# reesque/SfmFromScratch

Measured on AMD Instinct MI355X. Metric: images/sec detect+describe+match, 1080p, 1/2/4/8 MI355X, higher is better.
Workload: dtype f32; 1 GPU; BASELINE configs[1]: 32x 1080p per GPU, ScaleRotInvSIFT 4-level x2 octave pyramid, k=2500, fw 18, NNRatio 0.85 over consecutive pairs; frames_per_gpu=32, pairs_per_gpu=31, distinct_batches=2, parallelism=image-shard x1, batches_in_flight=2

## Files before the change

include/sfmfeat.h:

```cpp
#ifndef SFMFEAT_H_
#define SFMFEAT_H_

#include <stddef.h>
#include <stdint.h>

#ifdef __cplusplus
extern "C" {
#endif

#define SFM_OK 0
#define SFM_EINVAL 1
#define SFM_ESTATE 2
#define SFM_EDEVICE 3
#define SFM_ERANGE 4
#define SFM_EINDEX 5

#define SFM_MODE_SCALEROT 0
#define SFM_MODE_NAIVE 1

#define SFM_DESC_DIM 128
#define SFM_MAX_GAUSS 15
#define SFM_MAX_KSIZE 31
#define SFM_MAX_FW 64
#define SFM_MAX_LEVELS 12
// ... 215 lines not shown
#define SFM_GEOM_COMPOSE 4
#define SFM_GEOM_ROTATE 5
#define SFM_GEOM_WAVE_SUM 6
#define SFM_GEOM_BLOCK_SUM 7
#define SFM_GEOM_OPS 8
int32_t sfm_debug_geom(int32_t device, int32_t op, const double* in, int64_t n, double* out);

int32_t sfm_debug_nms(int32_t device, const float* R, int32_t B, int32_t H, int32_t W, int32_t ksize,
                      const uint32_t* tnms, int32_t tile, uint64_t* keys_out, int64_t* counts_out);

#define SFM_SELECT_STATE_WORDS 11
#define SFM_SELECT_CONSTS 5
int32_t sfm_debug_select(int32_t device, int32_t nlevels, int32_t B, const float* const* R, const int32_t* H,
                         const int32_t* W, const int32_t* half_window, int32_t k, int32_t ksize, int64_t vmin,
                         int32_t force_exact, int32_t* x, int32_t* y, float* conf, int32_t* count,
                         uint32_t* state, int64_t* ncand, int32_t* consts);

float sfm_debug_time_harris(int32_t device, int32_t abl, int32_t B, int32_t H, int32_t W,
                            int32_t iters);
float sfm_debug_harris_stamps(int32_t device, int32_t abl, int32_t B, int32_t H, int32_t W,
                              int32_t iters, uint64_t* out, int64_t cap);

int64_t sfm_debug_match_stamps(uint64_t* out, int64_t cap);

int32_t sfm_debug_match_operands(sfm_ctx* ctx, int32_t slot, int64_t rows, uint16_t* hi, uint16_t* lo,
                                 float* norm2, float* rnorm, float* pmax);
int32_t sfm_debug_match_windows(sfm_ctx* ctx, int32_t pair, int64_t rows, int32_t* cand_n, float* cand_thr,
                                uint32_t* cand);
int32_t sfm_debug_match_skips(sfm_ctx* ctx, int32_t pair, int64_t rows, uint8_t* skip);

int32_t sfm_copy_wg(void* dst, const void* src, int64_t bytes, int32_t workgroups, void* stream);

int32_t sfm_debug_select_stats(sfm_ctx* ctx, int32_t* fallback_planes, int32_t* total_planes);
int32_t sfm_debug_pose_candidates(sfm_ctx* ctx, int32_t* cand_idx, int64_t entries);
int32_t sfm_debug_ransac_fits(sfm_ctx* ctx, double* F, int32_t* counts, int64_t entries);
int32_t sfm_debug_pnp_fits(sfm_ctx* ctx, double* hyp, int32_t* counts, double* start_Rt, int64_t entries);
int32_t sfm_debug_copy_level(sfm_ctx* ctx, int32_t l, int32_t what, float* out, void* stream);
int64_t sfm_debug_bmax_stride(int32_t h, int32_t w);
void sfm_debug_set_nms_blocks(int32_t mode);
int32_t sfm_debug_nms_blocks_rule(int32_t h, int32_t w, int32_t kcap, int32_t ksize);
int32_t sfm_debug_nms_blocks(int32_t device, const float* R, int32_t B, int32_t H, int32_t W, const uint32_t* tnms,
                             const uint32_t* fallback, int32_t blocks, int32_t inflate, uint64_t* keys_out,
                             int64_t* counts_out);


#ifdef __cplusplus
}
#endif

#endif
```

sfmfromscratch_amd/_native.py:

```python
from __future__ import annotations

import ctypes
import os
import sys
import threading

import numpy as np

from . import _abi
from ._abi import SfmParams

_HERE = os.path.dirname(os.path.abspath(__file__))
LIB_PATH = os.environ.get("SFMFEAT_LIB", os.path.join(_HERE, "lib", "libsfmfeat.so"))

_lib = None
_lib_lock = threading.Lock()

_fp = ctypes.POINTER(ctypes.c_float)
_i64p = ctypes.POINTER(ctypes.c_int64)
_i32p = ctypes.POINTER(ctypes.c_int32)
_u8p = ctypes.POINTER(ctypes.c_uint8)
_dp = ctypes.POINTER(ctypes.c_double)
_vp = ctypes.c_void_p

# ... 56 lines not shown
                                               _vp, _vp, _vp, _vp, _vp, _vp, ctypes.c_double, _vp, _vp, _vp]),
    "sfm_resect_tracks_dev": (ctypes.c_int32, [_vp, _vp, _vp, ctypes.c_int32, ctypes.c_int64, _vp, _vp,
                                               ctypes.c_int32, _vp, _vp, ctypes.c_int32, ctypes.c_double,
                                               ctypes.c_int32, ctypes.c_int64, ctypes.c_int32, _vp, _vp, _vp, _vp,
                                               _vp, _vp, _vp]),
    "sfm_ingest_rgb_dev": (ctypes.c_int32, [_vp, _vp, ctypes.c_int32, ctypes.c_int32, ctypes.c_int32,
                                            ctypes.c_int32, ctypes.c_int32, _vp, _vp]),
    "sfm_extract_batch_dev": (ctypes.c_int32, [_vp, _vp, ctypes.c_int32, ctypes.c_int32, ctypes.c_int32, _vp, _vp,
                                               _vp, ctypes.c_int64, _vp]),
    "sfm_extract_batch_u8_dev": (ctypes.c_int32, [_vp, _vp, ctypes.c_int32, ctypes.c_int32, ctypes.c_int32, _vp,
                                                  _vp, _vp, ctypes.c_int64, _vp]),
    "sfm_match_pairs_dev": (ctypes.c_int32, [_vp, _vp, _vp, ctypes.c_int32, ctypes.c_int64, _vp, ctypes.c_int32,
                                             ctypes.c_float, _vp, _vp, _vp, _vp]),
    "sfm_match_prep_dev": (ctypes.c_int32, [_vp, _vp, _vp, ctypes.c_int32, ctypes.c_int64, ctypes.c_int32,
                                            ctypes.c_int32, _vp]),
    "sfm_match_pairs_prepped_dev": (ctypes.c_int32, [_vp, _vp, _vp, ctypes.c_int32, ctypes.c_int64, _vp,
                                                     ctypes.c_int32, ctypes.c_float, _vp, _vp, _vp, _vp]),
    "sfm_ctx_stream": (ctypes.c_int32, [_vp, ctypes.POINTER(_vp)]),
    "sfm_ctx_set_serial": (ctypes.c_int32, [_vp, ctypes.c_int32]),
    "sfm_ctx_set_fused_prep": (ctypes.c_int32, [_vp, ctypes.c_int32]),
    "sfm_ctx_set_priority": (ctypes.c_int32, [_vp, ctypes.c_int32]),
    "sfm_gate_create": (ctypes.c_int32, [ctypes.c_int32, ctypes.POINTER(_vp)]),
    "sfm_gate_destroy": (ctypes.c_int32, [_vp]),
    "sfm_ctx_set_gate": (ctypes.c_int32, [_vp, _vp]),
    "sfm_profile_enable": (ctypes.c_int32, [_vp, ctypes.c_int32]),
    "sfm_profile_stages": (ctypes.c_int32, [_vp, ctypes.c_int32]),
    "sfm_profile_read": (ctypes.c_int32, [_vp, ctypes.POINTER(ctypes.c_double), _i64p, ctypes.c_int32]),
    "sfm_profile_spans": (ctypes.c_int32, [_vp, ctypes.c_int64]),
    "sfm_profile_spans_read": (ctypes.c_int32, [_vp, _i64p, _i32p, ctypes.c_int64, _i64p, _i64p, ctypes.c_int32]),
    "sfm_debug_time_harris": (ctypes.c_float, [ctypes.c_int32] * 6),
    "sfm_debug_harris_stamps": (ctypes.c_float, [ctypes.c_int32] * 6 + [ctypes.c_void_p, ctypes.c_int64]),
    "sfm_debug_match_stamps": (ctypes.c_int64, [ctypes.c_void_p, ctypes.c_int64]),
    "sfm_debug_select_stats": (ctypes.c_int32, [_vp, _i32p, _i32p]),
    **_abi.MATCH_DEBUG_SIGNATURES,
    **_abi.GEOM_DEBUG_SIGNATURES,
    **_abi.SELECT_DEBUG_SIGNATURES,
    **_abi.PNP_DEBUG_SIGNATURES,
    "sfm_copy_wg": (ctypes.c_int32, [_vp, _vp, ctypes.c_int64, ctypes.c_int32, _vp]),
    "sfm_dist_unique_id": (ctypes.c_int32, [_u8p]),
    "sfm_dist_create": (ctypes.c_int32, [ctypes.c_int32, ctypes.c_int32, ctypes.c_int32, _u8p, ctypes.POINTER(_vp)]),
    "sfm_dist_destroy": (ctypes.c_int32, [_vp]),
    "sfm_dist_last_error": (ctypes.c_char_p, [_vp]),
    "sfm_dist_rank": (ctypes.c_int32, [_vp, _i32p, _i32p]),
    "sfm_dist_allgather_slots_dev": (ctypes.c_int32, [_vp, ctypes.c_int32, ctypes.c_int32, _vp, _vp, _vp, _vp, _vp,
                                                      _vp, ctypes.c_int64, _vp]),
    "sfm_dist_halo_dev": (ctypes.c_int32, [_vp, ctypes.c_int32, _vp, _vp, _vp, _vp, _vp, _vp, _vp]),

    "sfm_debug_copy_level": (ctypes.c_int32, [_vp, ctypes.c_int32, ctypes.c_int32, _vp, _vp]),
    "sfm_debug_atan2": (ctypes.c_int32, [ctypes.c_int32, _fp, _fp, _fp, ctypes.c_int64]),
    "sfm_debug_harris": (ctypes.c_int32, [ctypes.c_int32, _fp, ctypes.c_int32, ctypes.c_double, ctypes.c_int32,
                                          _fp, ctypes.c_int32, ctypes.c_int32, _fp, _fp, _i64p]),
    "sfm_debug_nms": (ctypes.c_int32, [ctypes.c_int32, _fp, ctypes.c_int32, ctypes.c_int32, ctypes.c_int32,
                                       ctypes.c_int32, _vp, ctypes.c_int32, _vp, _i64p]),
    "sfm_debug_bmax_stride": (ctypes.c_int64, [ctypes.c_int32, ctypes.c_int32]),
    "sfm_debug_set_nms_blocks": (None, [ctypes.c_int32]),
    "sfm_debug_nms_blocks_rule": (ctypes.c_int32, [ctypes.c_int32] * 4),
    "sfm_debug_nms_blocks": (ctypes.c_int32, [ctypes.c_int32, _fp, ctypes.c_int32, ctypes.c_int32, ctypes.c_int32,
                                              _vp, _vp, ctypes.c_int32, ctypes.c_int32, _vp, _i64p]),
}


class NativeLibraryMissing(ImportError):
    pass


def _preload_torch_hip_runtime():
# ... 94 lines not shown
            raise RuntimeError("sfm_ctx_create failed: no usable MI355X (HIP) device")
        self.handle = h
        self.capacity = int(self.lib.sfm_keypoint_capacity(ctypes.byref(params)))
        self.levels = 1 if params.mode == _abi.SFM_MODE_NAIVE else int(params.pyramid_level)

    def close(self):
        if getattr(self, "handle", None) is not None and self.handle.value:
            self.lib.sfm_ctx_destroy(self.handle)
            self.handle = _vp()

    def __del__(self):
        try:
            self.close()
        except Exception:
            pass

    def stream(self) -> int:
        h = _vp()
        check(self.lib.sfm_ctx_stream(self.handle, ctypes.byref(h)), self.handle)
        return int(h.value or 0)

    def set_priority(self, priority: int):
        check(self.lib.sfm_ctx_set_priority(self.handle, int(priority)), self.handle)

    def set_fused_prep(self, on: bool):
        check(self.lib.sfm_ctx_set_fused_prep(self.handle, 1 if on else 0), self.handle)

    def set_serial(self, serial: bool):
        check(self.lib.sfm_ctx_set_serial(self.handle, 1 if serial else 0), self.handle)

    def select_stats(self):
        fb, tot = ctypes.c_int32(0), ctypes.c_int32(0)
        check(self.lib.sfm_debug_select_stats(self.handle, ctypes.byref(fb), ctypes.byref(tot)), self.handle)
        return int(fb.value), int(tot.value)

    def copy_level(self, level: int, what: int, out_ptr: int, stream: int):
        check(self.lib.sfm_debug_copy_level(self.handle, int(level), int(what), ctypes.c_void_p(out_ptr),
                                            ctypes.c_void_p(stream)), self.handle)

    def extract(self, img: np.ndarray):
        if img.dtype != np.float32:
            img = img.astype(np.float32)
        if img.strides[1] != 4:
            img = np.ascontiguousarray(img)
        H, W = img.shape
        cap = max(self.capacity, 1)
        X = np.empty(cap, np.int64)
        Y = np.empty(cap, np.int64)
        D = np.empty((cap, 128), np.float32)
        C = np.empty(cap, np.float32)
        lc = np.zeros(self.levels, np.int32)
        n = ctypes.c_int64(0)
        rc = self.lib.sfm_extract(self.handle, img.ctypes.data_as(_fp), H, W, img.strides[0] // 4,
                                  X.ctypes.data_as(_i64p), Y.ctypes.data_as(_i64p), D.ctypes.data_as(_fp),
                                  C.ctypes.data_as(_fp), cap, ctypes.byref(n), lc.ctypes.data_as(_i32p))
        check(rc, self.handle)
        k = n.value
        return X[:k], Y[:k], D[:k], C[:k], lc

    def match(self, d1: np.ndarray, d2: np.ndarray, ratio32: np.float32):
        d1 = np.ascontiguousarray(d1, dtype=np.float32)
        d2 = np.ascontiguousarray(d2, dtype=np.float32)
        n1, n2 = d1.shape[0], d2.shape[0]
        cap = max(n1, 1)
        m = np.empty((cap, 2), np.int64)
        c = np.empty(cap, np.float32)
# ... 306 lines not shown
    nc = ctypes.c_int64(0)
    check(load_library().sfm_debug_harris(device, g.ctypes.data_as(_fp), gs, params.alpha, params.ksize,
                                          img.ctypes.data_as(_fp), H, W, R.ctypes.data_as(_fp),
                                          med.ctypes.data_as(_fp), ctypes.byref(nc)))
    return R, med[0], nc.value


def debug_nms(R: np.ndarray, tnms, ksize: int = 3, tile: bool = False, device: int = 0):
    R = np.ascontiguousarray(R, dtype=np.float32)
    B, H, W = R.shape
    t = np.ascontiguousarray(tnms, dtype=np.uint32)
    keys = np.zeros(B * H * W, np.uint64)
    cnt = np.zeros(B, np.int64)
    check(load_library().sfm_debug_nms(device, R.ctypes.data_as(_fp), B, H, W, ksize, t.ctypes.data,
                                       int(tile), keys.ctypes.data, cnt.ctypes.data_as(_i64p)))
    return [np.sort(keys[b * H * W: b * H * W + cnt[b]]) for b in range(B)]


def debug_nms_blocks(R: np.ndarray, tnms, fallback=None, blocks: bool = True, inflate: bool = False, device: int = 0):
    R = np.ascontiguousarray(R, dtype=np.float32)
    B, H, W = R.shape
    t = np.ascontiguousarray(tnms, dtype=np.uint32)
    fb = np.zeros(B, np.uint32) if fallback is None else np.ascontiguousarray(fallback, dtype=np.uint32)
    assert t.shape == (B,) and fb.shape == (B,)
    keys = np.zeros(B * H * W, np.uint64)
    cnt = np.zeros(B, np.int64)
    check(load_library().sfm_debug_nms_blocks(device, R.ctypes.data_as(_fp), B, H, W, t.ctypes.data, fb.ctypes.data,
                                              int(blocks), int(inflate), keys.ctypes.data, cnt.ctypes.data_as(_i64p)))
    return [np.sort(keys[b * H * W: b * H * W + cnt[b]]) for b in range(B)]


def set_nms_blocks(mode: int):
    load_library().sfm_debug_set_nms_blocks(int(mode))


def nms_blocks_rule(h: int, w: int, kcap: int, ksize: int = 3) -> bool:
    return bool(load_library().sfm_debug_nms_blocks_rule(int(h), int(w), int(kcap), int(ksize)))


def bmax_stride(h: int, w: int) -> int:
    return int(load_library().sfm_debug_bmax_stride(int(h), int(w)))


def debug_geom(op: int, rows: np.ndarray, device: int = 0) -> np.ndarray:
    op = int(op)
    if not 0 <= op < len(_abi.GEOM_ROW_IN):
        raise ValueError(f"debug_geom: unknown op {op}")
    if not isinstance(rows, np.ndarray) or rows.dtype != np.float64 or not rows.flags.c_contiguous:
        raise ValueError("debug_geom: rows must be a C-contiguous float64 array")
    if rows.ndim != 2 or rows.shape[1] != _abi.GEOM_ROW_IN[op]:
        raise ValueError(f"debug_geom: op {op} takes rows of {_abi.GEOM_ROW_IN[op]} values, got shape {rows.shape}")
    n = rows.shape[0]
    if n > _abi.SFM_GEOM_MAX_ROWS:
        raise ValueError(f"debug_geom: at most {_abi.SFM_GEOM_MAX_ROWS} rows")
    out = np.empty((n, _abi.GEOM_ROW_OUT[op]), np.float64)
    if n:
        check(load_library().sfm_debug_geom(device, op, rows.ctypes.data, n, out.ctypes.data))
    return out


def select_constants(k: int) -> dict:
    consts = np.zeros(_abi.SFM_SELECT_CONSTS, np.int32)
    check(load_library().sfm_debug_select(0, 0, 0, None, None, None, None, int(k), 1, 0, 0, None, None, None, None,
                                          None, None, consts.ctypes.data))
    return dict(zip(_abi.SELECT_CONST_FIELDS, consts.tolist()))

# ... 147 lines not shown
```

sfmfromscratch_amd/csrc/api_extract.hip:

```cpp
#include "ctx.h"

using namespace sfm;

static_assert(kLayoutMedBins == kMedBins1 && kLayoutCounterStride == kCounterStride &&
                  kLayoutMedianStateBytes == sizeof(MedianState) && kLayoutSelectMaxLevels == kSelectMaxLevels,
              "extract_layout.h mirrors kernels.h");
static_assert(layout_bmax_stride(1080, 1920) == bmax_plane_stride(1080, 1920) &&
                  layout_bmax_stride(270, 480) == bmax_plane_stride(270, 480) &&
                  layout_bmax_stride(70, 132) == bmax_plane_stride(70, 132),
              "extract_layout.h mirrors kernels.h");

static int g_nms_blocks_override = -2;
void extract_set_nms_blocks(int mode) { g_nms_blocks_override = mode < -1 ? -2 : mode; }

LayoutSwitches extract_layout_switches() {
  LayoutSwitches s = extract_switches().layout;
  if (g_nms_blocks_override != -2) s.nms_blocks = g_nms_blocks_override;
  return s;
}

const ExtractSwitches& extract_switches() {
  static const ExtractSwitches sw = [] {
    ExtractSwitches s;
    s.layout.pyr_fused = env_int(getenv("SFMFEAT_PYR_FUSED"), 1) != 0;
// ... 112 lines not shown
    const float alpha = (float)c->p.alpha;
    if (!(l0 > 0 && (skip & 16))) launch_harris_levels(g, B, as<float>(c->ex.gauss), c->p.gaussian_size, alpha, st);
  }

  void select_level(int l, hipStream_t s) {
    StageScope sc(c, SFM_PROF_TOPK, s);
    if (skip & 1) return;
    launch_select(R(l), cand(l), candcnt + y.counter[l], at<uint32_t>(kBufMedlist, y.sel[l]),
                  at<uint64_t>(kBufScratch, y.sel[l]), kp(l), std::max(c->kcap, 1), c->kcap, B, y.lv[l].h, y.lv[l].w,
                  c->p.ksize, y.lv[l].fw / 2, med(l), s);
  }

  void select_merged() {
    StageScope sc(c, SFM_PROF_TOPK, st);
    SelectLevels g{};
    g.n = y.L - y.L_aux;
    for (int l = y.L_aux; l < y.L; ++l)
      g.l[l - y.L_aux] = SelectLevels::Level{R(l), cand(l), candcnt + y.counter[l], at<uint32_t>(kBufMedlist, y.sel[l]),
                                             at<uint64_t>(kBufScratch, y.sel[l]), kp(l), med(l), y.lv[l].h, y.lv[l].w,
                                             y.lv[l].fw / 2};
    if (!(skip & 1)) launch_select_levels(g, std::max(c->kcap, 1), c->kcap, B, c->p.ksize, st);
  }

  void describe_level(int l, hipStream_t s) {
    StageScope sc(c, SFM_PROF_DESCRIBE, s);
    const int L = y.L;
    if ((skip & 2) && l != L - 1) {
      fused_ok = false;
      return;
    }
    bool ow = false;
    const bool r = launch_describe(lvl[l], B, y.lv[l].h, y.lv[l].w, y.lv[l].fw, c->p.mode == SFM_MODE_NAIVE ? 0 : 1,
                                   kp(l), c->kcap, as<int32_t>(c->ex.buf[kBufLc]), l, L, y.lv[l].scale, xy, desc, conf,
                                   cap, l == L - 1 ? count : nullptr, mo, &ow, s);
    if (l == L - 1) counted = r;
    fused_ok = fused_ok && ow;
  }

  int release_gate() {
    if (c->gate && !gate_released) {
      HIPCHK(c, hipEventRecord(c->gate->ev, st));
      c->gate->armed = true;
      gate_released = true;
    }
    return SFM_OK;
  }

  int run(const float* imgs);
};

int Extraction::run(const float* imgs) {
  const int L = y.L, L_aux = y.L_aux;
  CtxStreams& cs = c->s;
  int rc;
  lvl[0] = imgs;
  for (int l = 1; l < L; ++l) lvl[l] = at<float>(kBufLvl, y.lvl[l]);
  zeroed = sw.fill_launches;
  {
    StageScope sc(c, SFM_PROF_PYRAMID, st);
    if (!y.pyr_fused) pyramid_from(1);
  }
  if ((rc = operands_fused_begin(c, desc, count, cap, B, &mo))) return rc;
  if (mo.hi) HIPCHK(c, hipMemsetAsync(mo.pmax, 0, (size_t)B * match_pmax_bytes(mo.capP), st));
  fused_ok = mo.hi != nullptr;
  if (!zeroed || sw.fill_launches) {
    HIPCHK(c, hipMemsetAsync(c->ex.buf[kBufHist].p, 0, y.bytes[kBufHist], st));
    HIPCHK(c, hipMemsetAsync(c->ex.buf[kBufCounts].p, 0, y.bytes[kBufCounts], st));
// ... 158 lines not shown
```

sfmfromscratch_amd/csrc/api_profile.hip:

```cpp
#include "ctx.h"

using namespace sfm;

namespace {

int spans_reset(sfm_ctx* c) {
  ProfilerWs& pr = c->prof;
  pr.span_n = 0;
  pr.span_dropped = 0;
  pr.span_level.clear();
  if (pr.span_cap == 0) return SFM_OK;
  std::vector<unsigned long long> init((size_t)2 * pr.span_cap, 0ull);
  for (int64_t i = 0; i < pr.span_cap; ++i) init[2 * i] = ~0ull;
  HIPCHK(c, hipDeviceSynchronize());
  HIPCHK(c, hipMemcpy(pr.spans.p, init.data(), init.size() * 8, hipMemcpyHostToDevice));
  return SFM_OK;
}

}

extern "C" {

int32_t sfm_profile_enable(sfm_ctx* c, int32_t on) {
  if (!c) return SFM_EINVAL;
// ... 72 lines not shown
int32_t sfm_debug_copy_level(sfm_ctx* c, int32_t l, int32_t what, float* out, void* stream) {
  if (!c || !out || l < 0 || l >= c->L || !c->ex.last_B) return SFM_EINVAL;
  ExtractWs& x = c->ex;
  ExtractLayout y;
  if (extract_layout(&c->p, c->kcap, x.last_B, x.last_H, x.last_W, c->serial, extract_layout_switches(), &y) != SFM_OK)
    return SFM_EINVAL;
  if (what == 2) {
    if (!((x.last_mapped >> l) & 1u) || y.bmax[l] < 0) return set_err(c, SFM_EINVAL, "the level wrote no block-maximum map");
    HIPCHK(c, hipMemcpyAsync(out, as<float>(x.buf[kBufBmax]) + y.bmax[l],
                             (size_t)x.last_B * bmax_plane_stride(y.lv[l].h, y.lv[l].w) * 4, hipMemcpyDeviceToDevice,
                             (hipStream_t)stream));
    return SFM_OK;
  }
  const size_t bytes = (size_t)x.last_B * y.lv[l].h * y.lv[l].w * 4;
  const float* src = what == 0 ? as<float>(x.buf[kBufR]) + y.plane[l]
                               : (l == 0 ? as<float>(x.buf[kBufImg0]) : as<float>(x.buf[kBufLvl]) + y.lvl[l]);
  HIPCHK(c, hipMemcpyAsync(out, src, bytes, hipMemcpyDeviceToDevice, (hipStream_t)stream));
  return SFM_OK;
}

int32_t sfm_debug_select_stats(sfm_ctx* c, int32_t* fallback_planes, int32_t* total_planes) {
  if (!c || !fallback_planes || !total_planes) return SFM_EINVAL;
  *fallback_planes = 0;
  *total_planes = c->L * c->ex.last_B;
  if (*total_planes == 0) return SFM_OK;
  HIPCHK(c, hipSetDevice(c->device));
  HIPCHK(c, hipDeviceSynchronize());
  std::vector<MedianState> ms((size_t)*total_planes);
  HIPCHK(c, hipMemcpy(ms.data(), c->ex.buf[kBufMed].p, ms.size() * sizeof(MedianState), hipMemcpyDeviceToHost));
  for (const MedianState& m : ms) *fallback_planes += m.fallback ? 1 : 0;
  return SFM_OK;
}

}
```

sfmfromscratch_amd/csrc/debug.hip:

```cpp
#include <string.h>

#include <vector>

#include "../../include/sfmfeat.h"
#include "kernels.h"

using namespace sfm;

namespace sfm {

__global__ void k_debug_atan2(const float* __restrict__ y, const float* __restrict__ x,
                              float* __restrict__ out, int64_t n) {
  int64_t i = (int64_t)blockIdx.x * blockDim.x + threadIdx.x;
  if (i < n) out[i] = svml_atan2f(y[i], x[i]);
}

__global__ void __launch_bounds__(256) k_copy_wg(const uint4* __restrict__ src, uint4* __restrict__ dst, int64_t n16,
                                                 const uint8_t* __restrict__ src_b, uint8_t* __restrict__ dst_b,
                                                 int64_t tail) {
  const int64_t stride = (int64_t)gridDim.x * blockDim.x;
  for (int64_t i = (int64_t)blockIdx.x * blockDim.x + threadIdx.x; i < n16; i += stride) dst[i] = src[i];
  if (blockIdx.x == 0 && threadIdx.x < tail) dst_b[threadIdx.x] = src_b[threadIdx.x];
}

// ... 122 lines not shown
    x = x * 1664525u + 1013904223u;
    h[i] = (float)(x >> 24) / 255.0f;
  }
  float g0[49];
  for (int i = 0; i < 49; ++i) g0[i] = 1.0f / 49.0f;
  std::vector<float> g(harris_taps_floats(7));
  harris_taps_build(g0, 7, g.data());
  (void)hipMemcpy(d_img, h.data(), n * 4, hipMemcpyHostToDevice);
  (void)hipMemcpy(d_g, g.data(), 4 * g.size(), hipMemcpyHostToDevice);
  (void)hipMemset(d_hist, 0, (size_t)B * 4 * kMedBins1);
  float ms = time_harris_ablation(abl, d_img, d_R, d_hist, B, H, W, d_g, 0.05f, iters, d_st, d_st ? cap : 0);
  if (d_st) {
    (void)hipMemcpy(out, d_st, (size_t)cap * 8, hipMemcpyDeviceToHost);
    (void)hipFree(d_st);
  }
  void* bufs[] = {d_img, d_R, d_g, d_hist};
  for (void* b : bufs) (void)hipFree(b);
  return ms;
}

int32_t sfm_copy_wg(void* dst, const void* src, int64_t bytes, int32_t workgroups, void* stream) {
  if (bytes < 0 || workgroups < 1 || (bytes > 0 && (!dst || !src))) return SFM_EINVAL;
  if ((((uintptr_t)dst) | ((uintptr_t)src)) & 15) return SFM_EINVAL;
  if (bytes == 0) return SFM_OK;
  const int64_t n16 = bytes / 16, tail = bytes - 16 * n16;
  hipLaunchKernelGGL(k_copy_wg, dim3((unsigned)workgroups), dim3(256), 0, (hipStream_t)stream,
                     (const uint4*)src, (uint4*)dst, n16, (const uint8_t*)src + 16 * n16, (uint8_t*)dst + 16 * n16,
                     tail);
  return hipGetLastError() == hipSuccess ? SFM_OK : SFM_EDEVICE;
}

int64_t sfm_debug_match_stamps(uint64_t* out, int64_t cap) { return sfm::match_stamps_copy(out, cap); }

}
```

sfmfromscratch_amd/csrc/describe.hip:

```cpp
#include "kernels.h"

#include <stdlib.h>

namespace sfm {

SFM_DEV double pi_edge(int i, int num) {
  const double start = -3.141592653589793, stop = 3.141592653589793;
  if (i == num - 1) return stop;
  double step = (stop - start) / (double)(num - 1);
  return (double)i * step + start;
}

struct DescLayout {
  int ws, n, n4, pw, P;
  size_t off_keys, off_patch, off_ori, off_mag, off_sw, off_cw, off_cellw, off_wgh, total;
};

__host__ __device__ inline DescLayout desc_layout(int fw, int rotate) {
  DescLayout L;
  int h = fw / 2;
  L.ws = 2 * h;
  L.n = L.ws * L.ws;
  L.pw = L.ws + 2;
  int P = 1;
// ... 231 lines not shown
  float v0 = w0, v1 = w1;
  if (nrm > 0.0f) {
    v0 = v0 / nrm;
    v1 = v1 / nrm;
  }
  out_desc[slot * 128 + lane] = sqrtf(v0);
  out_desc[slot * 128 + lane + 64] = sqrtf(v1);
  if (lane == 0) {
    if (out_conf) out_conf[slot] = kp.conf[ko];
    out_xy[slot * 2 + 0] = (int32_t)((double)x * scale);
    out_xy[slot * 2 + 1] = (int32_t)((double)y * scale);
  }
}

__global__ void k_finalize_counts(const int32_t* __restrict__ lc_all, int B, int L,
                                  int32_t* __restrict__ out_count) {
  int b = blockIdx.x * blockDim.x + threadIdx.x;
  if (b >= B) return;
  int32_t s = 0;
  for (int l = 0; l < L; ++l) s += lc_all[(int64_t)l * B + b];
  out_count[b] = s;
}

size_t describe_lds_bytes(int fw, int rotate) { return desc_layout(fw, rotate).total; }

void init_describe_attributes(size_t max_lds) {
  (void)hipFuncSetAttribute((const void*)k_describe, hipFuncAttributeMaxDynamicSharedMemorySize,
                            (int)max_lds);
}

bool launch_describe(const float* lvl, int B, int H, int W, int fw, int rotate, KpList kp,
                     int kcap, const int32_t* level_counts_all, int level, int L, double scale,
                     int32_t* out_xy, float* out_desc, float* out_conf, int64_t out_cap,
                     int32_t* out_count, const MatchOperands& mo, bool* operands_written, hipStream_t st) {
  if (operands_written) *operands_written = false;
  if (kcap <= 0) return false;
  static const bool one_per_wave = [] {
    const char* v = getenv("SFMFEAT_DESCRIBE");
    return v && v[0] == 'w';
  }();
  if (!one_per_wave && launch_describe_quad(lvl, B, H, W, fw, rotate, kp, kcap, level_counts_all, level,
                                            scale, out_xy, out_desc, out_conf, out_cap, out_count, L, mo, st)) {
    if (operands_written) *operands_written = mo.hi != nullptr;
    return out_count != nullptr;
  }
  size_t lds = describe_lds_bytes(fw, rotate);
  hipLaunchKernelGGL(k_describe, dim3(kcap, B), dim3(64), lds, st, lvl, H, W, fw, rotate, kp, kcap,
                     level_counts_all, level, B, scale, out_xy, out_desc, out_conf, out_cap);
  return false;
}

void launch_finalize_counts(const int32_t* level_counts_all, int B, int L, int32_t* out_count,
                            hipStream_t st) {
  hipLaunchKernelGGL(k_finalize_counts, dim3((B + 255) / 256), dim3(256), 0, st, level_counts_all, B, L,
                     out_count);
}

}
```

sfmfromscratch_amd/csrc/describe_q.hip:

```cpp
#include "kernels.h"

#include <stdlib.h>
#include <string.h>

#include <mutex>

namespace sfm {
namespace dq {

constexpr int cmax(int a, int b) { return a > b ? a : b; }
constexpr int pow2ceil(int v) { return v <= 1 ? 1 : 2 * pow2ceil((v + 1) / 2); }

template <int WS, int ROT>
struct Geo {
  static constexpr int N = WS * WS, PW = WS + 2, NP = PW * PW;
  static constexpr int P = cmax(pow2ceil(N), 16), E = P / 16;
  static constexpr int RN = (N + 15) / 16;
  static constexpr int A = (cmax(cmax(NP, N + 4), 16 * 17) + 3) & ~3;
  static constexpr int NQ = (N + 3) & ~3;
  static constexpr int OFF_M = A;
  static constexpr int OFF_K = OFF_M + NQ;
  static constexpr int OFF_R = OFF_K + NQ;
  static constexpr int OFF_I = OFF_R + (ROT ? (NQ / 2 + 3) & ~3 : 0);
  static constexpr int OFF_T = OFF_I + (ROT ? 40 : 0);
  static constexpr int G = OFF_T + 12;
};

SFM_DEV double pi_edge(int i, int num) {
  const double start = -3.141592653589793, stop = 3.141592653589793;
  if (i == num - 1) return stop;
  const double step = (stop - start) / (double)(num - 1);
  return (double)i * step + start;
}
// ... 113 lines not shown
  gy = __builtin_fmaf(-2.0f, a01, gy);
  gy = __builtin_fmaf(-1.0f, a02, gy);
  gy = __builtin_fmaf(1.0f, a20, gy);
  gy = __builtin_fmaf(2.0f, a21, gy);
  gy = __builtin_fmaf(1.0f, a22, gy);
  const float sx = gx * gx;
  const float sy = gy * gy;
  const float s = sx + sy;
  mag = sqrtf(s);
  ori = svml_atan2f(gy, gx);
}

SFM_DEV void cas_up(uint32_t& a, uint32_t& b) {
  const uint32_t lo = min(a, b), hi = max(a, b);
  a = lo;
  b = hi;
}

template <typename T>
SFM_DEV void batcher16(T (&q)[16]) {
#pragma unroll
  for (int p = 1; p < 16; p <<= 1)
#pragma unroll
    for (int kk = p; kk >= 1; kk >>= 1)
#pragma unroll
      for (int j = kk % p; j + kk < 16; j += 2 * kk)
#pragma unroll
        for (int i = 0; i < kk; ++i) {
          const int a = i + j, c = i + j + kk;
          if (c < 16 && a / (2 * p) == c / (2 * p)) cas_up(q[a], q[c]);
        }
}

template <int WS, int ROT, int ABL = 0>
__global__ void __launch_bounds__(64) k_describe_q(const float* __restrict__ lvl, int H, int W, KpList kp,
                                                   int kcap, const int32_t* __restrict__ lc_all, int level,
                                                   int B, double scale, int32_t* __restrict__ out_xy,
                                                   float* __restrict__ out_desc, float* __restrict__ out_conf,
                                                   int64_t out_cap, int32_t* __restrict__ out_count, int L,
                                                   MatchOperands mo) {
  using C = Geo<WS, ROT>;
  constexpr int N = C::N, PW = C::PW, NP = C::NP, E = C::E, RN = C::RN, h = WS / 2;
  __shared__ __attribute__((aligned(16))) float s_all[4 * C::G];
  const int b = blockIdx.y;
  if (out_count != nullptr && blockIdx.x == 0 && threadIdx.x == 0) {
    int32_t s = 0;
    for (int l = 0; l < L; ++l) s += lc_all[(int64_t)l * B + b];
    out_count[b] = s;
  }
  const int nkb = (kcap + 3) / 4;
  if ((int)blockIdx.x >= nkb) {
    int32_t s = 0;
    for (int l = 0; l < L; ++l) s += lc_all[(int64_t)l * B + b];
    const int nt = ((int)gridDim.x - nkb) * 64;
    for (int64_t r = s + ((int)blockIdx.x - nkb) * 64 + threadIdx.x; r < mo.capP; r += nt) {
      const int64_t mr = (int64_t)b * mo.capP + r;
      uint4* hz = reinterpret_cast<uint4*>(mo.hi + mr * 128);
      uint4* lz = reinterpret_cast<uint4*>(mo.lo + mr * 128);
#pragma unroll
      for (int q = 0; q < 16; ++q) {
        hz[q] = make_uint4(0u, 0u, 0u, 0u);
        lz[q] = make_uint4(0u, 0u, 0u, 0u);
      }
      mo.norm2[mr] = INFINITY;
      mo.rnorm[mr] = 0.0f;
    }
    return;
  }
  const int count = kp.count[b];
  const int kbase = blockIdx.x * 4;
  if (kbase >= count) return;
  const int lane = threadIdx.x, g = lane >> 4, gl = lane & 15;
  const int kpi = kbase + g;
  const bool valid = kpi < count;
  const int64_t ko = (int64_t)b * kcap + (valid ? kpi : kbase);
  const int x = kp.x[ko], y = kp.y[ko];
  float* sA = s_all + g * C::G;
  float* sM = sA + C::OFF_M;
  uint32_t* sK = reinterpret_cast<uint32_t*>(sA + C::OFF_K);
  uint16_t* sR = reinterpret_cast<uint16_t*>(sA + C::OFF_R);
  int32_t* sI = reinterpret_cast<int32_t*>(sA + C::OFF_I);
  uint32_t* sT = reinterpret_cast<uint32_t*>(sA + C::OFF_T);

  const float* img = lvl + (int64_t)b * H * W;
#pragma unroll
  for (int it = 0; it < (NP + 15) / 16; ++it) {
    const int e0 = it * 16 + gl;
    const int e = e0 < NP ? e0 : NP - 1;
    const int pr = e / PW, pc = e - pr * PW;
    const int gy = y - h + pr, gx = x - h + pc;
    const bool in = gy >= 0 && gy < H && gx >= 0 && gx < W;
    const int cy = min(max(gy, 0), H - 1), cx = min(max(gx, 0), W - 1);
    const float v = (ABL & 64) ? (float)(cy + cx) : img[(int64_t)cy * W + cx];
    if (e0 < NP) sA[e] = in ? v : 0.0f;
  }
  __syncthreads();

  double k[E];
  bool tiny = false;
#pragma unroll
  for (int r = 0; r < E; ++r) k[r] = __longlong_as_double((long long)kPad);
#pragma unroll
  for (int r = 0; r < RN; ++r) {
    const int e0 = r * 16 + gl;
    const bool ok = (N % 16 == 0) || e0 < N;
    const int e = ok ? e0 : N - 1;
    const int i = e / WS, j = e - i * WS;
    float mag, ori;
    if constexpr ((ABL & 8) != 0) {
      mag = sA[(i + 1) * PW + (j + 1)];
      ori = sA[(i + 1) * PW + j] - 100.0f;
    } else {
      grad_at(sA + (i + 1) * PW + (j + 1), PW, mag, ori);
    }
    if (ok) {
      sM[e] = mag;
      if (!ROT) sK[e] = __float_as_uint(ori);
    }
    if (ROT) {
      k[r] = ok ? dkey(((uint64_t)fkey(ori) << 9) | (uint32_t)e) : __longlong_as_double((long long)kPad);
      tiny |= ok && ori != 0.0f && fabsf(ori) < 0x1p-25f;
    }
  }
  __syncthreads();

  double dom = 0.0;
  int dom_bin = 36;
  if constexpr (ROT) {
    if constexpr ((ABL & 1) == 0) merge_level<E, 2>(k, gl);
    float w[E];
    uint32_t ke[E], kf[E];
#pragma unroll
    for (int r = 0; r < E; ++r) {
      const int p = gl * E + r;
      const uint64_t pl = dpayload(k[r]);
      ke[r] = p < N ? (uint32_t)(pl & 511u) : 0u;
      kf[r] = (uint32_t)(pl >> 9);
      w[r] = p < N ? sM[ke[r]] : 0.0f;
    }
    __syncthreads();
    float cw[E];
#pragma unroll
    for (int r = 0; r < E; ++r) cw[r] = 0.0f;
    float carry = 0.0f;
    constexpr int NL = (N + E - 1) / E;
    if constexpr ((ABL & 2) != 0) {
#pragma unroll
      for (int r = 0; r < E; ++r) cw[r] = w[r];
    }
    for (int s = 0; s < ((ABL & 2) ? 0 : NL); ++s) {
      if (gl == s) {
        float acc = carry;
#pragma unroll
        for (int r = 0; r < E; ++r) {
          acc = acc + w[r];
          cw[r] = acc;
        }
      }
      const float nxt = __uint_as_float(dpp<0x111>(__float_as_uint(cw[E - 1])));
      if (gl == s + 1) carry = nxt;
    }
// ... 44 lines not shown
    for (int t = 0; t < 3; ++t) {
      const int j = gl + 16 * t;
      if (j < 36) {
        const float v = sA[3 + sI[j + 1]] - sA[3 + sI[j]];
        if (v > hb) { hb = v; bi = j; }
      }
    }
    {
      float ov; int oi;
      ov = rxorf<8>(hb); oi = (int)rxor<8>((uint32_t)bi);
      if (ov > hb || (ov == hb && oi < bi)) { hb = ov; bi = oi; }
      ov = rxorf<4>(hb); oi = (int)rxor<4>((uint32_t)bi);
      if (ov > hb || (ov == hb && oi < bi)) { hb = ov; bi = oi; }
      ov = rxorf<2>(hb); oi = (int)rxor<2>((uint32_t)bi);
      if (ov > hb || (ov == hb && oi < bi)) { hb = ov; bi = oi; }
      ov = rxorf<1>(hb); oi = (int)rxor<1>((uint32_t)bi);
      if (ov > hb || (ov == hb && oi < bi)) { hb = ov; bi = oi; }
    }
    dom = (pi_edge(bi, 37) + pi_edge(bi + 1, 37)) / 2.0;
    dom_bin = bi;
  }

  if (gl < 9) sT[gl] = (ABL & 32) ? 0x80000000u + (uint32_t)(dom * 1e6) * gl : c_cell[dom_bin][gl];
  __syncthreads();
  float hv[8];
  if constexpr ((ABL & 4) != 0) {
#pragma unroll
    for (int bb = 0; bb < 8; ++bb) hv[bb] = sM[gl * 8 + bb] + __uint_as_float(sT[bb & 7]);
  } else {
  const int r4 = gl >> 2, c4 = gl & 3;
  float wv[16];
  uint32_t hk[16];
  const bool grp_tiny = ROT && ((__ballot(tiny) >> (16 * g)) & 0xFFFFull) != 0;
  if (ROT && !grp_tiny) {
    uint32_t q[16];
#pragma unroll
    for (int t = 0; t < 16; ++t) {
      const int i = 4 * r4 + (t >> 2), j = 4 * c4 + (t & 3);
      const bool ok = i < WS && j < WS;
      q[t] = ok ? (uint32_t)sR[ok ? i * WS + j : 0] : 0xFFFFFFFFu;
    }
    batcher16(q);
#pragma unroll
    for (int m = 0; m < 16; ++m) {
      const bool ok = q[m] != 0xFFFFFFFFu;
      const uint32_t p = ok ? q[m] : 0u;
      wv[m] = ok ? sM[p] : 0.0f;
      hk[m] = ok ? sK[p] : 0xFFFFFFFFu;
    }
  } else {
    uint64_t q[16];
#pragma unroll
    for (int t = 0; t < 16; ++t) {
      const int i = 4 * r4 + (t >> 2), j = 4 * c4 + (t & 3);
      const bool ok = i < WS && j < WS;
      const int e = ok ? i * WS + j : 0;
      const uint32_t key = ROT ? sK[sR[e]] : fkey(__uint_as_float(sK[e]));
      q[t] = ok ? (((uint64_t)key << 32) | (uint32_t)t) : ~0ull;
    }
    if (!ROT) {
      double dq16[16];
#pragma unroll
      for (int t = 0; t < 16; ++t) dq16[t] = q[t] == ~0ull ? __longlong_as_double((long long)kPad)
                                                           : dkey(((q[t] >> 32) << 4) | (uint32_t)t);
      batcher16(dq16);
#pragma unroll
      for (int t = 0; t < 16; ++t) {
// ... 130 lines not shown
namespace {
uint32_t fkey_h(float v) {
  uint32_t b;
  memcpy(&b, &v, 4);
  if (b == 0x80000000u) b = 0u;
  return (b & 0x80000000u) ? ~b : (b | 0x80000000u);
}
float fkey_inv_h(uint32_t k) {
  const uint32_t b = (k & 0x80000000u) ? (k & 0x7fffffffu) : ~k;
  float f;
  memcpy(&f, &b, 4);
  return f;
}
double pi_edge_h(int i, int num) {
  const double start = -3.141592653589793, stop = 3.141592653589793;
  if (i == num - 1) return stop;
  const double step = (stop - start) / (double)(num - 1);
  return (double)i * step + start;
}
uint32_t edge_key_h(double e, double sh, bool strict) {
  auto pass = [&](uint32_t kk) {
    const double d = (double)fkey_inv_h(kk) - sh;
    return strict ? d > e : d >= e;
  };
  uint32_t lo = fkey_h(-INFINITY), hi = fkey_h(INFINITY);
  while (hi - lo > 1u) {
    const uint32_t mid = lo + (hi - lo) / 2u;
    if (pass(mid)) hi = mid; else lo = mid;
  }
  return hi;
}
}

void init_describe_quad_tables() {
  static std::mutex mu;
  static bool done[256] = {};
  int dev = 0;
  if (hipGetDevice(&dev) != hipSuccess || dev < 0 || dev >= 256) return;
  std::lock_guard<std::mutex> lk(mu);
  if (done[dev]) return;
  uint32_t ori[37], cell[37][9];
  for (int j = 0; j < 37; ++j) ori[j] = edge_key_h(pi_edge_h(j, 37), 0.0, j == 36);
  for (int bi = 0; bi < 37; ++bi) {
    const double dom = bi < 36 ? (pi_edge_h(bi, 37) + pi_edge_h(bi + 1, 37)) / 2.0 : 0.0;
    for (int t = 0; t < 9; ++t) cell[bi][t] = edge_key_h(pi_edge_h(t, 9), dom, t == 8);
  }
  done[dev] = hipMemcpyToSymbol(HIP_SYMBOL(dq::c_ori), ori, sizeof(ori)) == hipSuccess &&
              hipMemcpyToSymbol(HIP_SYMBOL(dq::c_cell), cell, sizeof(cell)) == hipSuccess;
}

#define SFM_DQ_BODY(WS)                                                                              \
    if (rotate)                                                                                      \
      hipLaunchKernelGGL((dq::k_describe_q<WS, 1>), grid, dim3(64), 0, st, lvl, H, W, kp, kcap, lc,  \
                         level, B, scale, out_xy, out_desc, out_conf, out_cap, out_count, L, mo);        \
    else                                                                                             \
      hipLaunchKernelGGL((dq::k_describe_q<WS, 0>), grid, dim3(64), 0, st, lvl, H, W, kp, kcap, lc,  \
                         level, B, scale, out_xy, out_desc, out_conf, out_cap, out_count, L, mo);        \
    return true;
#define SFM_DQ_CASE(WS) \
  case WS:              \
    SFM_DQ_BODY(WS)

bool launch_describe_quad(const float* lvl, int B, int H, int W, int fw, int rotate, KpList kp, int kcap,
                          const int32_t* lc, int level, double scale, int32_t* out_xy, float* out_desc,
                          float* out_conf, int64_t out_cap, int32_t* out_count, int L, const MatchOperands& mo,
                          hipStream_t st) {
  constexpr int kPadBlocks = 8;
  const dim3 grid((kcap + 3) / 4 + (mo.hi != nullptr && out_count != nullptr ? kPadBlocks : 0), B);
  switch (2 * (fw / 2)) {
    SFM_DQ_CASE(2)
    SFM_DQ_CASE(4)
    SFM_DQ_CASE(6)
    SFM_DQ_CASE(8)
    SFM_DQ_CASE(10)
    SFM_DQ_CASE(12)
    SFM_DQ_CASE(14)
    SFM_DQ_CASE(16)
    case 18:
#ifdef SFM_ABLATIONS
      if (rotate) {
        static const int abl = [] {
          const char* v = SFM_ABLATION_ENV("SFMFEAT_DQ_ABL");
          return v ? atoi(v) : 0;
        }();
        switch (abl) {
#define SFM_DQ_ABL(A)                                                                                     \
  case A:                                                                                                \
    hipLaunchKernelGGL((dq::k_describe_q<18, 1, A>), grid, dim3(64), 0, st, lvl, H, W, kp, kcap, lc, level, \
                       B, scale, out_xy, out_desc, out_conf, out_cap, out_count, L, mo);                     \
    return true;
          SFM_DQ_ABL(1)
          SFM_DQ_ABL(2)
          SFM_DQ_ABL(4)
          SFM_DQ_ABL(8)
          SFM_DQ_ABL(7)
          SFM_DQ_ABL(16)
          SFM_DQ_ABL(32)
          SFM_DQ_ABL(64)
          SFM_DQ_ABL(55)
          SFM_DQ_ABL(127)
          default:
            break;
        }
      }
#endif
      SFM_DQ_BODY(18)
    SFM_DQ_CASE(20)
    SFM_DQ_CASE(22)
    default:
      return false;
  }
}

}
```

sfmfromscratch_amd/csrc/kernels.h:

```cpp
#pragma once

#include <hip/hip_runtime.h>
#include <stdint.h>

#include <vector>

#include "common.h"

namespace sfm {

#define SFM_NMS_MAX_HALF 15

constexpr int kHistBits = 12;
constexpr int kHistBins = 1 << kHistBits;
constexpr int kMedBits1 = 11;
constexpr int kMedBins1 = 1 << kMedBits1;
constexpr int kTopkLdsCap = 8192;
constexpr int kMaxMatchRows = 16384;
constexpr int kMatchCandCap = 256;
constexpr int kCounterStride = 32;
constexpr int kMatchUnitPairBits = 20;

constexpr float kMatchScale = 256.0f;
constexpr float kMatchLoScale = 2048.0f;
// ... 327 lines not shown

void launch_nms(const float* R, const MedianState* state, uint64_t* cand,
                unsigned long long* cand_count, int B, int H, int W, int ksize, int mode, hipStream_t st,
                int force_tile = 0, const float* bmax = nullptr);
bool nms_blocks_shape(int W, int ksize, int mode);

void init_topk_attributes();
void init_describe_attributes(size_t max_lds);
void init_describe_quad_tables();
size_t describe_lds_bytes(int fw, int rotate);
void launch_select(const float* R, uint64_t* cand, const unsigned long long* cand_count, uint32_t* medlist,
                   uint64_t* scratch, KpList kp, int kcap, int k, int B, int H, int W, int ksize, int half_window,
                   MedianState* state, hipStream_t st);
constexpr int kSelectMaxLevels = 4;
struct SelectLevels {
  struct Level {
    const float* R;
    uint64_t* cand;
    const unsigned long long* cand_count;
    uint32_t* medlist;
    uint64_t* scratch;
    KpList kp;
    MedianState* state;
    int H, W, hw;
  } l[kSelectMaxLevels];
  int n;
};
void launch_select_levels(const SelectLevels& g, int kcap, int k, int B, int ksize, hipStream_t st);
void select_branch_sizes(int k, int32_t out[5]);

bool launch_describe_quad(const float* lvl, int B, int H, int W, int fw, int rotate, KpList kp, int kcap,
                          const int32_t* level_counts_all, int level, double scale, int32_t* out_xy,
                          float* out_desc, float* out_conf, int64_t out_cap, int32_t* out_count, int L,
                          const MatchOperands& mo, hipStream_t st);
bool launch_describe(const float* lvl, int B, int H, int W, int fw, int rotate, KpList kp,
                     int kcap, const int32_t* level_counts_all, int level, int L, double scale,
                     int32_t* out_xy, float* out_desc, float* out_conf, int64_t out_cap,
                     int32_t* out_count, const MatchOperands& mo, bool* operands_written, hipStream_t st);
void launch_finalize_counts(const int32_t* level_counts_all, int B, int L, int32_t* out_count,
                            hipStream_t st);

struct RowBest {
  int32_t col;
  float nndr;
};
SFM_DEV void top2_update(float d, int j, float& e1, int& j1, float& e2) {
  if (d < e1 || (d == e1 && j < j1)) {
    e2 = e1;
    e1 = d;
    j1 = j;
  } else if (d < e2) {
    e2 = d;
  }
}
SFM_DEV void top2_merge(float& e1, int& j1, float& e2, float o1, int oj, float o2) {
  if (o1 < e1 || (o1 == e1 && oj < j1)) {
    e2 = fminf(e1, o2);
    e1 = o1;
    j1 = oj;
  } else {
    e2 = fminf(e2, o1);
  }
}
SFM_DEV RowBest top2_finish(float e1, int j1, float e2, float ratio) {
  RowBest rb;
  rb.col = -1;
  rb.nndr = 0.0f;
  const float d1 = sqrtf(e1), d2 = sqrtf(e2);
  if (d2 > 0.0f) {
    const float nndr = d1 / d2;
    if (nndr <= ratio) { rb.col = j1; rb.nndr = nndr; }
// ... 23 lines not shown
```

Before: 45080 images/sec.

## Certify dominant orientation via LDS histogram, skip full sort when margin safe

For rotation-invariant describe at widths 4 and 20+, each keypoint group builds a 36-bin orientation histogram in shared memory with atomics and finds the top two bins. If the gap between them exceeds a rounding-error bound for every group in the wave, the dominant bin is taken directly and the full merge-sort over all patch samples is skipped. Otherwise it falls back to the original sorted path and bumps a fallback counter. This adds histogram atomics, LDS traffic and a new per-cell sort on the fast path, and only applies to certain window widths.

```diff
diff --git a/include/sfmfeat.h b/include/sfmfeat.h
--- a/include/sfmfeat.h
+++ b/include/sfmfeat.h
@@ -271,6 +271,10 @@
 int32_t sfm_copy_wg(void* dst, const void* src, int64_t bytes, int32_t workgroups, void* stream);
 
 int32_t sfm_debug_select_stats(sfm_ctx* ctx, int32_t* fallback_planes, int32_t* total_planes);
+#define SFM_DESCRIBE_CERT_C 8
+#define SFM_DESCRIBE_CERT_TMIN_EXP (-64)
+void sfm_debug_set_describe_cert(int32_t mode);
+int32_t sfm_debug_describe_stats(sfm_ctx* ctx, int64_t* fallback_groups, int64_t* groups);
 int32_t sfm_debug_pose_candidates(sfm_ctx* ctx, int32_t* cand_idx, int64_t entries);
 int32_t sfm_debug_ransac_fits(sfm_ctx* ctx, double* F, int32_t* counts, int64_t entries);
 int32_t sfm_debug_pnp_fits(sfm_ctx* ctx, double* hyp, int32_t* counts, double* start_Rt, int64_t entries);
diff --git a/sfmfromscratch_amd/_native.py b/sfmfromscratch_amd/_native.py
--- a/sfmfromscratch_amd/_native.py
+++ b/sfmfromscratch_amd/_native.py
@@ -112,6 +112,8 @@
     "sfm_debug_harris_stamps": (ctypes.c_float, [ctypes.c_int32] * 6 + [ctypes.c_void_p, ctypes.c_int64]),
     "sfm_debug_match_stamps": (ctypes.c_int64, [ctypes.c_void_p, ctypes.c_int64]),
     "sfm_debug_select_stats": (ctypes.c_int32, [_vp, _i32p, _i32p]),
+    "sfm_debug_set_describe_cert": (None, [ctypes.c_int32]),
+    "sfm_debug_describe_stats": (ctypes.c_int32, [_vp, _i64p, _i64p]),
     **_abi.MATCH_DEBUG_SIGNATURES,
     **_abi.GEOM_DEBUG_SIGNATURES,
     **_abi.SELECT_DEBUG_SIGNATURES,
@@ -272,6 +274,11 @@
     def select_stats(self):
         fb, tot = ctypes.c_int32(0), ctypes.c_int32(0)
         check(self.lib.sfm_debug_select_stats(self.handle, ctypes.byref(fb), ctypes.byref(tot)), self.handle)
+        return int(fb.value), int(tot.value)
+
+    def describe_stats(self):
+        fb, tot = ctypes.c_int64(0), ctypes.c_int64(0)
+        check(self.lib.sfm_debug_describe_stats(self.handle, ctypes.byref(fb), ctypes.byref(tot)), self.handle)
         return int(fb.value), int(tot.value)
 
     def copy_level(self, level: int, what: int, out_ptr: int, stream: int):
@@ -644,6 +651,10 @@
 
 def set_nms_blocks(mode: int):
     load_library().sfm_debug_set_nms_blocks(int(mode))
+
+
+def set_describe_cert(mode: int):
+    load_library().sfm_debug_set_describe_cert(int(mode))
 
 
 def nms_blocks_rule(h: int, w: int, kcap: int, ksize: int = 3) -> bool:
diff --git a/sfmfromscratch_amd/csrc/api_extract.hip b/sfmfromscratch_amd/csrc/api_extract.hip
--- a/sfmfromscratch_amd/csrc/api_extract.hip
+++ b/sfmfromscratch_amd/csrc/api_extract.hip
@@ -168,7 +168,7 @@
     bool ow = false;
     const bool r = launch_describe(lvl[l], B, y.lv[l].h, y.lv[l].w, y.lv[l].fw, c->p.mode == SFM_MODE_NAIVE ? 0 : 1,
                                    kp(l), c->kcap, as<int32_t>(c->ex.buf[kBufLc]), l, L, y.lv[l].scale, xy, desc, conf,
-                                   cap, l == L - 1 ? count : nullptr, mo, &ow, s);
+                                   cap, l == L - 1 ? count : nullptr, mo, &ow, donecnt + y.counter[l], s);
     if (l == L - 1) counted = r;
     fused_ok = fused_ok && ow;
   }
diff --git a/sfmfromscratch_amd/csrc/api_profile.hip b/sfmfromscratch_amd/csrc/api_profile.hip
--- a/sfmfromscratch_amd/csrc/api_profile.hip
+++ b/sfmfromscratch_amd/csrc/api_profile.hip
@@ -128,4 +128,31 @@
   return SFM_OK;
 }
 
+int32_t sfm_debug_describe_stats(sfm_ctx* c, int64_t* fallback_groups, int64_t* groups) {
+  if (!c || !fallback_groups || !groups) return SFM_EINVAL;
+  *fallback_groups = *groups = 0;
+  ExtractWs& x = c->ex;
+  if (!x.last_B || c->p.mode == SFM_MODE_NAIVE) return SFM_OK;
+  ExtractLayout y;
+  if (extract_layout(&c->p, c->kcap, x.last_B, x.last_H, x.last_W, c->serial, extract_layout_switches(), &y) != SFM_OK)
+    return SFM_EINVAL;
+  HIPCHK(c, hipSetDevice(c->device));
+  HIPCHK(c, hipDeviceSynchronize());
+  const int B = x.last_B, L = y.L;
+  std::vector<int32_t> lc((size_t)L * B);
+  std::vector<unsigned long long> cnt((size_t)y.counter_block);
+  HIPCHK(c, hipMemcpy(lc.data(), x.buf[kBufLc].p, lc.size() * 4, hipMemcpyDeviceToHost));
+  HIPCHK(c, hipMemcpy(cnt.data(), as<unsigned long long>(x.buf[kBufCounts]) + 3 * y.counter_block, cnt.size() * 8,
+                      hipMemcpyDeviceToHost));
+  for (int l = 0; l < L; ++l) {
+    const int ws = 2 * (y.lv[l].fw / 2);
+    if (ws < 2 || ws > 22) continue;
+    for (int b = 0; b < B; ++b) {
+      *groups += (lc[(size_t)l * B + b] + 3) / 4;
+      *fallback_groups += (int64_t)cnt[(size_t)(y.counter[l] + (int64_t)b * kCounterStride + 1)];
+    }
+  }
+  return SFM_OK;
 }
+
+}
diff --git a/sfmfromscratch_amd/csrc/debug.hip b/sfmfromscratch_amd/csrc/debug.hip
--- a/sfmfromscratch_amd/csrc/debug.hip
+++ b/sfmfromscratch_amd/csrc/debug.hip
@@ -178,4 +178,6 @@
 
 int64_t sfm_debug_match_stamps(uint64_t* out, int64_t cap) { return sfm::match_stamps_copy(out, cap); }
 
+void sfm_debug_set_describe_cert(int32_t mode) { describe_set_cert(mode); }
+
 }
diff --git a/sfmfromscratch_amd/csrc/describe.hip b/sfmfromscratch_amd/csrc/describe.hip
--- a/sfmfromscratch_amd/csrc/describe.hip
+++ b/sfmfromscratch_amd/csrc/describe.hip
@@ -287,7 +287,8 @@
 bool launch_describe(const float* lvl, int B, int H, int W, int fw, int rotate, KpList kp,
                      int kcap, const int32_t* level_counts_all, int level, int L, double scale,
                      int32_t* out_xy, float* out_desc, float* out_conf, int64_t out_cap,
-                     int32_t* out_count, const MatchOperands& mo, bool* operands_written, hipStream_t st) {
+                     int32_t* out_count, const MatchOperands& mo, bool* operands_written,
+                     unsigned long long* fb_count, hipStream_t st) {
   if (operands_written) *operands_written = false;
   if (kcap <= 0) return false;
   static const bool one_per_wave = [] {
@@ -295,7 +296,8 @@
     return v && v[0] == 'w';
   }();
   if (!one_per_wave && launch_describe_quad(lvl, B, H, W, fw, rotate, kp, kcap, level_counts_all, level,
-                                            scale, out_xy, out_desc, out_conf, out_cap, out_count, L, mo, st)) {
+                                            scale, out_xy, out_desc, out_conf, out_cap, out_count, L, mo, fb_count,
+                                            st)) {
     if (operands_written) *operands_written = mo.hi != nullptr;
     return out_count != nullptr;
   }
diff --git a/sfmfromscratch_amd/csrc/describe_q.hip b/sfmfromscratch_amd/csrc/describe_q.hip
--- a/sfmfromscratch_amd/csrc/describe_q.hip
+++ b/sfmfromscratch_amd/csrc/describe_q.hip
@@ -1,4 +1,5 @@
 #include "kernels.h"
+#include "../../include/sfmfeat.h"
 
 #include <stdlib.h>
 #include <string.h>
@@ -178,16 +179,23 @@
         }
 }
 
+constexpr float kCertBoundPerN = (float)SFM_DESCRIBE_CERT_C * 0x1p-24f;
+constexpr uint32_t kCertTminBits = (uint32_t)(127 + SFM_DESCRIBE_CERT_TMIN_EXP) << 23;
+constexpr bool cert_width(int ws) { return ws == 4 || ws >= 20; }
+
 template <int WS, int ROT, int ABL = 0>
 __global__ void __launch_bounds__(64) k_describe_q(const float* __restrict__ lvl, int H, int W, KpList kp,
                                                    int kcap, const int32_t* __restrict__ lc_all, int level,
                                                    int B, double scale, int32_t* __restrict__ out_xy,
                                                    float* __restrict__ out_desc, float* __restrict__ out_conf,
                                                    int64_t out_cap, int32_t* __restrict__ out_count, int L,
-                                                   MatchOperands mo) {
+                                                   MatchOperands mo, int cert,
+                                                   unsigned long long* __restrict__ fb_count) {
   using C = Geo<WS, ROT>;
   constexpr int N = C::N, PW = C::PW, NP = C::NP, E = C::E, RN = C::RN, h = WS / 2;
+  constexpr bool CERT = ROT && (ABL == 128 || (ABL == 0 && cert_width(WS)));
   __shared__ __attribute__((aligned(16))) float s_all[4 * C::G];
+  __shared__ uint32_t s_ori[CERT ? 40 : 1];
   const int b = blockIdx.y;
   if (out_count != nullptr && blockIdx.x == 0 && threadIdx.x == 0) {
     int32_t s = 0;
@@ -226,6 +234,7 @@
   uint32_t* sK = reinterpret_cast<uint32_t*>(sA + C::OFF_K);
   uint16_t* sR = reinterpret_cast<uint16_t*>(sA + C::OFF_R);
   int32_t* sI = reinterpret_cast<int32_t*>(sA + C::OFF_I);
+  float* sH = sA + C::OFF_I;
   uint32_t* sT = reinterpret_cast<uint32_t*>(sA + C::OFF_T);
 
   const float* img = lvl + (int64_t)b * H * W;
@@ -240,12 +249,16 @@
     const float v = (ABL & 64) ? (float)(cy + cx) : img[(int64_t)cy * W + cx];
     if (e0 < NP) sA[e] = in ? v : 0.0f;
   }
+  if constexpr (CERT) {
+    if (lane < 37) s_ori[lane] = c_ori[lane];
+    sH[gl] = 0.0f;
+    sH[gl + 16] = 0.0f;
+    if (gl < 4) sH[gl + 32] = 0.0f;
+  }
   __syncthreads();
 
-  double k[E];
   bool tiny = false;
-#pragma unroll
-  for (int r = 0; r < E; ++r) k[r] = __longlong_as_double((long long)kPad);
+  float tsum = 0.0f;
 #pragma unroll
   for (int r = 0; r < RN; ++r) {
     const int e0 = r * 16 + gl;
@@ -261,18 +274,63 @@
     }
     if (ok) {
       sM[e] = mag;
-      if (!ROT) sK[e] = __float_as_uint(ori);
-    }
-    if (ROT) {
-      k[r] = ok ? dkey(((uint64_t)fkey(ori) << 9) | (uint32_t)e) : __longlong_as_double((long long)kPad);
-      tiny |= ok && ori != 0.0f && fabsf(ori) < 0x1p-25f;
+      sK[e] = ROT ? fkey(ori) : __float_as_uint(ori);
+    }
+    if (ROT) tiny |= ok && ori != 0.0f && fabsf(ori) < 0x1p-25f;
+    if constexpr (CERT) {
+      const uint32_t fk = fkey(ori);
+      const float t = (ori + __uint_as_float(0x40490fdbu)) * 5.729578f;
+      const int b0 = min(max((int)t, 0), 35);
+      const int bb = b0 - (fk < s_ori[b0] ? 1 : 0) + (fk >= s_ori[b0 + 1] ? 1 : 0);
+      if ((ABL & 128) == 0 && ok && bb >= 0 && bb < 36) atomicAdd(&sH[bb], mag);
+      if ((ABL & 128) != 0 && bb == 36) sH[0] = mag;
+      tsum += ok ? mag : 0.0f;
     }
   }
   __syncthreads();
 
   double dom = 0.0;
   int dom_bin = 36;
-  if constexpr (ROT) {
+  bool fast = false;
+  if constexpr (CERT) {
+    float h1 = -1.0f, h2 = -1.0f;
+    int bi = 0;
+#pragma unroll
+    for (int t = 0; t < 3; ++t) {
+      const int j = gl + 16 * t;
+      if (j < 36) {
+        const float v = sH[j];
+        if (v > h1) { h2 = h1; h1 = v; bi = j; } else if (v > h2) { h2 = v; }
+      }
+    }
+    auto merge2 = [&](float o1, float o2, int oi) {
+      const float n2 = fmaxf(fminf(h1, o1), fmaxf(h2, o2));
+      if (o1 > h1) bi = oi;
+      h1 = fmaxf(h1, o1);
+      h2 = n2;
+    };
+    merge2(rxorf<8>(h1), rxorf<8>(h2), (int)rxor<8>((uint32_t)bi));
+    merge2(rxorf<4>(h1), rxorf<4>(h2), (int)rxor<4>((uint32_t)bi));
+    merge2(rxorf<2>(h1), rxorf<2>(h2), (int)rxor<2>((uint32_t)bi));
+    merge2(rxorf<1>(h1), rxorf<1>(h2), (int)rxor<1>((uint32_t)bi));
+    tsum = tsum + rxorf<8>(tsum);
+    tsum = tsum + rxorf<4>(tsum);
+    tsum = tsum + rxorf<2>(tsum);
+    tsum = tsum + rxorf<1>(tsum);
+    const uint32_t tb = __float_as_uint(tsum);
+    const bool certified = tb >= kCertTminBits && tb < 0x7f800000u && h1 - h2 > (kCertBoundPerN * (float)N) * tsum;
+    fast = (ABL & 128) != 0 || (cert != 0 && __ballot(certified && !tiny) == ~0ull);
+    if (fast) dom_bin = bi;
+  }
+  if (ROT && !fast) {
+    if (fb_count != nullptr && lane == 0) atomicAdd(fb_count + (int64_t)b * kCounterStride + 1, 1ull);
+    double k[E];
+#pragma unroll
+    for (int r = 0; r < E; ++r) {
+      const int e0 = r * 16 + gl;
+      const bool ok = r < RN && ((N % 16 == 0) || e0 < N);
+      k[r] = ok ? dkey(((uint64_t)sK[ok ? e0 : 0] << 9) | (uint32_t)e0) : __longlong_as_double((long long)kPad);
+    }
     if constexpr ((ABL & 1) == 0) merge_level<E, 2>(k, gl);
     float w[E];
     uint32_t ke[E], kf[E];
@@ -383,7 +441,24 @@
   float wv[16];
   uint32_t hk[16];
   const bool grp_tiny = ROT && ((__ballot(tiny) >> (16 * g)) & 0xFFFFull) != 0;
-  if (ROT && !grp_tiny) {
+  if (CERT && fast) {
+    double q[16];
+#pragma unroll
+    for (int t = 0; t < 16; ++t) {
+      const int i = 4 * r4 + (t >> 2), j = 4 * c4 + (t & 3);
+      const bool ok = i < WS && j < WS;
+      const int e = ok ? i * WS + j : 0;
+      q[t] = ok ? dkey(((uint64_t)sK[e] << 9) | (uint32_t)e) : __longlong_as_double((long long)kPad);
+    }
+    batcher16(q);
+#pragma unroll
+    for (int m = 0; m < 16; ++m) {
+      const uint64_t pl = dpayload(q[m]);
+      const bool ok = pl < (1ull << 41);
+      wv[m] = ok ? sM[ok ? (int)(pl & 511u) : 0] : 0.0f;
+      hk[m] = ok ? (uint32_t)(pl >> 9) : 0xFFFFFFFFu;
+    }
+  } else if (ROT && !grp_tiny) {
     uint32_t q[16];
 #pragma unroll
     for (int t = 0; t < 16; ++t) {
@@ -580,6 +655,9 @@
 }
 }
 
+static int g_describe_cert = 1;
+void describe_set_cert(int mode) { g_describe_cert = mode != 0 ? 1 : 0; }
+
 void init_describe_quad_tables() {
   static std::mutex mu;
   static bool done[256] = {};
@@ -600,10 +678,10 @@
 #define SFM_DQ_BODY(WS)                                                                              \
     if (rotate)                                                                                      \
       hipLaunchKernelGGL((dq::k_describe_q<WS, 1>), grid, dim3(64), 0, st, lvl, H, W, kp, kcap, lc,  \
-                         level, B, scale, out_xy, out_desc, out_conf, out_cap, out_count, L, mo);        \
+                         level, B, scale, out_xy, out_desc, out_conf, out_cap, out_count, L, mo, cert, fb_count);        \
     else                                                                                             \
       hipLaunchKernelGGL((dq::k_describe_q<WS, 0>), grid, dim3(64), 0, st, lvl, H, W, kp, kcap, lc,  \
-                         level, B, scale, out_xy, out_desc, out_conf, out_cap, out_count, L, mo);        \
+                         level, B, scale, out_xy, out_desc, out_conf, out_cap, out_count, L, mo, cert, fb_count);        \
     return true;
 #define SFM_DQ_CASE(WS) \
   case WS:              \
@@ -612,7 +690,8 @@
 bool launch_describe_quad(const float* lvl, int B, int H, int W, int fw, int rotate, KpList kp, int kcap,
                           const int32_t* lc, int level, double scale, int32_t* out_xy, float* out_desc,
                           float* out_conf, int64_t out_cap, int32_t* out_count, int L, const MatchOperands& mo,
-                          hipStream_t st) {
+                          unsigned long long* fb_count, hipStream_t st) {
+  const int cert = g_describe_cert;
   constexpr int kPadBlocks = 8;
   const dim3 grid((kcap + 3) / 4 + (mo.hi != nullptr && out_count != nullptr ? kPadBlocks : 0), B);
   switch (2 * (fw / 2)) {
@@ -635,7 +714,7 @@
 #define SFM_DQ_ABL(A)                                                                                     \
   case A:                                                                                                \
     hipLaunchKernelGGL((dq::k_describe_q<18, 1, A>), grid, dim3(64), 0, st, lvl, H, W, kp, kcap, lc, level, \
-                       B, scale, out_xy, out_desc, out_conf, out_cap, out_count, L, mo);                     \
+                       B, scale, out_xy, out_desc, out_conf, out_cap, out_count, L, mo, cert, fb_count);                     \
     return true;
           SFM_DQ_ABL(1)
           SFM_DQ_ABL(2)
@@ -647,6 +726,7 @@
           SFM_DQ_ABL(64)
           SFM_DQ_ABL(55)
           SFM_DQ_ABL(127)
+          SFM_DQ_ABL(128)
           default:
             break;
         }
diff --git a/sfmfromscratch_amd/csrc/kernels.h b/sfmfromscratch_amd/csrc/kernels.h
--- a/sfmfromscratch_amd/csrc/kernels.h
+++ b/sfmfromscratch_amd/csrc/kernels.h
@@ -383,11 +383,13 @@
 bool launch_describe_quad(const float* lvl, int B, int H, int W, int fw, int rotate, KpList kp, int kcap,
                           const int32_t* level_counts_all, int level, double scale, int32_t* out_xy,
                           float* out_desc, float* out_conf, int64_t out_cap, int32_t* out_count, int L,
-                          const MatchOperands& mo, hipStream_t st);
+                          const MatchOperands& mo, unsigned long long* fb_count, hipStream_t st);
+void describe_set_cert(int mode);
 bool launch_describe(const float* lvl, int B, int H, int W, int fw, int rotate, KpList kp,
                      int kcap, const int32_t* level_counts_all, int level, int L, double scale,
                      int32_t* out_xy, float* out_desc, float* out_conf, int64_t out_cap,
-                     int32_t* out_count, const MatchOperands& mo, bool* operands_written, hipStream_t st);
+                     int32_t* out_count, const MatchOperands& mo, bool* operands_written,
+                     unsigned long long* fb_count, hipStream_t st);
 void launch_finalize_counts(const int32_t* level_counts_all, int B, int L, int32_t* out_count,
                             hipStream_t st);
 
```

Result: slower. 44430 images/sec (-1.4%).
